# bwohlberg/sporco

Measured on AMD Instinct MI355X. Metric: ConvBPDN ADMM iterations/s, higher is better.
Workload: dtype f32; 1 GPU; admm.cbpdn.ConvBPDN 512x512 greyscale, K=64 8x8 filters, N=32 images per GPU, lambda=0.05, default options (AutoRho, stats every iteration); global_images=32, parallelism=image-shard x1

## Files before the change

sporco_amd/csrc/api_admm_run.inc:

```
    bool admm_run_supported(const sporco_amd_admm_params &p) const {
        return !cplx && std::is_same<T, float>::value && rows_ok && mr_ok(p) && (fused || fused_slabs) && !fused_mc &&
               !tail_mode && !(p.flags & (F_XRRS | F_GRADREG | F_KEEP_X | F_FEVAL_Y)) &&
               (!(p.flags & F_JOINT) || joint_rows_ok(p)) && p.lmbda >= 0.0 && p.rho > 0.0 &&
               !std::getenv("SPORCO_AMD_HOST_LOOP");
    }

    bool persist_ok(const sporco_amd_admm_params &p, const sporco_amd_admm_ctrl &c, bool vf,
                    bool has_reduce) const {
        const bool off = sw.persist >= 0 ? sw.persist != 1 : !hint_one_launch;
        return !off && vf && !has_reduce && fused && !fused_slabs && Ks == K && run_always_emit &&
               admm_persist_supported<T>(H, W, K) && !wl1.ptr && c.max_iter >= 3 &&
               !(p.flags & (F_NOBNDRY | F_AMS | F_JOINT)) && admm_persist_resident<T>(H, W, K, CN);
    }
    PersistIterArgs<T> persist_iter_args(const sporco_amd_admm_params &p, const T *vin, T *vout,
                                         double *prow, double *pcol) {
        PersistIterArgs<T> a;
        cx<T> *Xf = cv(SPORCO_AMD_VAR_XF);
        a.fwd.y = a.fwd.u = nullptr;
        a.fwd.v = vin;
        a.fwd.flags = p.flags;
        a.fwd.C = C;
        a.fwd.N = N;
        a.fwd.dH = p.dH;
        a.fwd.dW = p.dW;
// ... 14 lines not shown
        a.cols.twB = twB;
        a.cols.rho = (T)p.rho;
        a.cols.H = H;
        a.cols.W = W;
        a.cols.CN = CN;
        a.cols.K = K;
        a.cols.partials = pcol;
        a.cols.Ks = Ks;
        a.post.twA = twRows;
        a.post.t_next = Xf;
        a.post.t = Xf;
        a.post.twW = planW.tw<T>();
        a.post.y = a.post.u = nullptr;
        a.post.y_out = a.post.u_out = nullptr;
        a.post.v_in = vin;
        a.post.v_out = vout;
        a.post.x = nullptr;
        a.post.scale = T(1.0 / ((double)H * (double)W));
        a.post.rlx = (T)p.rlx;
        a.post.thr = T(0);
        a.post.u_scale = T(1);
        a.post.flags = p.flags;
        a.post.H = H;
        a.post.W = W;
        a.post.C = C;
        a.post.N = N;
        a.post.K = K;
        a.post.dH = p.dH;
        a.post.dW = p.dW;
        a.post.P = P;
        a.post.Ks = Ks;
        a.post.partials = prow;
        return a;
    }
    int run_persist(const sporco_amd_admm_params &p, int index0, int max_iter, T *v_prev, T *v_other,
                    bool want_sums) {
        const int grid = admm_persist_grid<T>(H, W, K, CN);
        const int64_t nrow = (int64_t)H * ceil_div(P, 128), ncol = (int64_t)Wf * CN;
        if (!pst_part_rows) {
            SA_HIP(hipMalloc((void **)&pst_part_rows, sizeof(double) * 8 * nrow));
            SA_HIP(hipMalloc((void **)&pst_part_f, sizeof(double) * 2 * ncol));
            SA_HIP(hipMalloc((void **)&pst_bar, sizeof(unsigned) * kPersistBarWords));
        }
        if (pst_grid < grid) {
            if (pst_blk) {
                sync();
                SA_HIP(hipFree(pst_blk));
                SA_HIP(hipFree(pst_ctl));
            }
            SA_HIP(hipMalloc(&pst_blk, sizeof(PersistIterArgs<T>) * 2 * grid));
            SA_HIP(hipMalloc((void **)&pst_ctl, sizeof(AdmmCtl) * grid));
            pst_grid = grid;
        }
        AdmmPersistArgs<T> a;
        const int p0 = index0 & 1;
        a.iter[p0] = persist_iter_args(p, v_prev, v_other, part_rows, part_f);
        a.iter[p0 ^ 1] = persist_iter_args(p, v_other, v_prev, pst_part_rows, pst_part_f);
        a.blk = static_cast<PersistIterArgs<T> *>(pst_blk);
        a.ctl_blk = pst_ctl;
        a.ctl = ctl_dev;
        a.rec = reinterpret_cast<AdmmRecord *>(rec_ring) + index0;
        a.index0 = index0;
        a.max_iter = max_iter - index0;
        a.bar = pst_bar;
        a.n_row_tiles = (int)nrow;
        a.n_col_tiles = (int)ncol;
        a.want_dfid = (p.flags & F_OBJ) ? 1 : 0;
        a.want_sums = want_sums ? 1 : 0;
        a.dfid_scale = 1.0 / ((double)H * W);
        SA_HIP(hipMemsetAsync(pst_bar, 0, sizeof(unsigned) * kPersistBarWords, st));
        {
            ProfScope ps(prof, PS_PERSIST);
            launch_admm_persist<T>(st, a, grid);
        }
        unsigned bar[16];
        SA_HIP(hipMemcpyAsync(bar, pst_bar, sizeof(bar), hipMemcpyDeviceToHost, st));
        sync();
        if (bar[2]) throw Error(SPORCO_AMD_EHIP, "one-launch solve: a grid barrier did not complete");
        xf_tiled = true;
        ++pst_runs;
        return (int)bar[3];
    }

    int64_t enqueue_iter_ctl(const sporco_amd_admm_params &p, const T *vin = nullptr,
                             T *vout = nullptr) {
        T *Y = vin ? nullptr : static_cast<T *>(vars[SPORCO_AMD_VAR_Y]);
        T *U = vin ? nullptr : static_cast<T *>(vars[SPORCO_AMD_VAR_U]);
        cx<T> *Xf = cv(SPORCO_AMD_VAR_XF);
        {
            RowsFwdArgs<T> ra;
            ra.y = Y;
            ra.u = U;
            ra.v = vin;
            ra.flags = p.flags;
            ra.C = C;
            ra.N = N;
            if (vin) {
                ra.wl1 = wl1;
                ra.dH = p.dH;
                ra.dW = p.dW;
                ra.ams_bits = ams_bits_of(p);
                ra.ams_k = Ku - 1;
            }
            ra.s2 = T(1);
            ra.t = Xf;
            ra.Ks = Ks;
            ra.twA = twRows;
            ra.H = H;
            ra.W = W;
            ra.CN = CN;
            ra.K = K;
            ra.P = P;
            ra.ctl = ctl_dev;
            ProfScope ps(prof, vin ? PS_ROWS_FWD_V : PS_ROWS_FWD);
            launch_rows_fwd<T>(st, ra);
        }
        {
            FusedColsArgs<T> fa;
            fa.t = Xf;
            fa.dft = dft;
            fa.sft = sft;
            fa.gramt = gramt;
            fa.twA = twA;
            fa.twB = twB;
            fa.rho = (T)p.rho;
            fa.H = H;
            fa.W = W;
            fa.CN = CN;
            fa.K = K;
            fa.partials = part_f;
            fa.Ks = Ks;
            fa.ctl = ctl_dev;
            if (cols_striped() && !fused_slabs) {
                fa.out_even = cols_out[0];
                fa.out_odd = cols_out[1];
            }
            ProfScope ps(prof, PS_FUSED_COLS);
            if (fused_slabs) {
                FusedSlabArgs<T> sa;
                sa.c = fa;
                sa.qpart = qpart;
                part_f_rows = (int)run_slab_cols(sa);
            } else {
                part_f_rows = (int)launch_fused_cols<T>(st, fa);
            }
            xf_tiled = true;
        }
        RowsPostArgs<T> pa;
        pa.twA = twRows;
        pa.t_next = nullptr;
        pa.t = Xf;
        if (cols_striped() && !fused_slabs) {
            pa.t = cols_out[0];
            pa.t_odd = cols_out[1];
        }
        pa.twW = planW.tw<T>();
        pa.y = Y;
        pa.u = U;
        pa.y_out = y_alt;
        pa.u_out = u_alt;
        pa.v_in = vin;
        pa.v_out = vout;
        pa.x = nullptr;
        pa.scale = T(1.0 / ((double)H * (double)W));
        pa.rlx = (T)p.rlx;
        pa.thr = T(0);
        pa.u_scale = T(1);
        pa.flags = p.flags;
        pa.H = H;
        pa.W = W;
        pa.C = C;
        pa.N = N;
        pa.K = K;
        pa.dH = p.dH;
        pa.dW = p.dW;
        pa.P = P;
        pa.wl1 = wl1;
        pa.Ks = Ks;
        pa.ams_bits = ams_bits_of(p);
        pa.ams_k = Ku - 1;
        pa.partials = part_rows;
        pa.ctl = ctl_dev;
        int64_t nt = 0;
        if (!run_always_emit) {
            ProfScope ps(prof, vin ? PS_ROWS_INV_POST_V : PS_ROWS_INV_POST);
            nt = launch_rows_inv_post<T>(st, pa);
        }
        pa.t_next = Xf;
        {
            ProfScope ps(prof, vin ? PS_ROWS_INV_POST_V_EMIT : PS_ROWS_INV_POST_EMIT);
            nt = launch_rows_inv_post<T>(st, pa);
        }
        if (!vout) {
            std::swap(vars[SPORCO_AMD_VAR_Y], reinterpret_cast<void *&>(y_alt));
            std::swap(vars[SPORCO_AMD_VAR_U], reinterpret_cast<void *&>(u_alt));
        }
        return nt;
    }

    int admm_run(const sporco_amd_admm_params &p, const sporco_amd_admm_ctrl &c,
                 sporco_amd_admm_record *records, double *rho_out, double *u_scale_out,
                 sporco_amd_reduce_fn reduce, void *user) override {
        require_ready();
        if (!admm_run_supported(p)) return -1;
        if (gv_live) ensure_yu();
        SA_REQUIRE(c.max_iter >= 0, "max_iter must not be negative");
        if (c.max_iter == 0) {
            *rho_out = p.rho;
            *u_scale_out = p.u_scale;
            return 0;
        }
        if (!y_alt) alloc_alt_pair();
        const bool nn = p.flags & F_NONNEG, jn = p.flags & F_JOINT;
        if (v_live && (!vform_ok(p) || !vform_same_opts(p))) ensure_yu();
        const bool vf = vform_ok(p) && (v_live || c.max_iter >= 4 || hint_vform);
        if (!vf) ensure_yu();
        const bool v_at_entry = v_live;
        T *const v_entry = v_cur;
        const T v_entry_thr = v_thr, v_entry_thr21 = v_thr21;
        if (!ctl_dev) SA_HIP(hipMalloc((void **)&ctl_dev, sizeof(AdmmCtl)));
        if (rec_cap < c.max_iter) {
            if (rec_ring) SA_HIP(hipHostFree(rec_ring));
            rec_cap = std::max(c.max_iter, 256);
            SA_HIP(hipHostMalloc((void **)&rec_ring, sizeof(AdmmRecord) * rec_cap, 0));
        }
        std::memset((void *)rec_ring, 0, sizeof(AdmmRecord) * c.max_iter);
        double *out_dev = out_dev_default;
        const bool want_sums = p.flags & (F_RESID | F_OBJ);
        AdmmCtlInit in;
        in.rho = p.rho;
        in.u_scale = p.u_scale;
        in.lmbda = p.lmbda;
        in.abstol = c.abs_tol;
        in.reltol = c.rel_tol;
        in.sqrt_nc = c.sqrt_nc;
        in.sqrt_nx = c.sqrt_nx;
        in.tau = c.rho_tau;
        in.mu = c.rho_mu;
        in.xi = c.rho_xi;
        in.mu21 = p.mu;
        in.k = c.k0;
        in.stable_run = stable_run;
        in.emitted = t_ready ? 1 : 0;
        in.is_f32 = 1;
        in.autorho = c.auto_rho;
        in.period = c.period > 0 ? c.period : 1;
        in.autoscaling = c.auto_scaling;
        in.stdres = c.std_residuals;
        in.need_resid = c.need_residuals;
        in.thr_prev = v_at_entry ? (float)v_entry_thr : 0.f;
        in.thr21_prev = v_at_entry ? (float)v_entry_thr21 : 0.f;
        in.no_speculation = sw.no_speculation ? 1 : 0;
        run_always_emit = !in.no_speculation && E <= ((int64_t)1 << 22);
        if (run_always_emit) in.no_speculation = 2;
        launch_admm_ctl_init(st, ctl_dev, in);
        SA_HIP(hipMemsetAsync(out_dev, 0, sizeof(double) * kOutSlots, st));
        const int ahead = c.lookahead > 0 ? c.lookahead : 3;
        int enq = 0, done = 0, stop_at = -1;
        int lag = std::getenv("SPORCO_AMD_RUN_LAG") ? std::atoi(std::getenv("SPORCO_AMD_RUN_LAG")) : 0;
        auto poll = [&](int upto, bool block) {
            while (done < upto && stop_at < 0) {
                if (rec_ring[done].seq != done + 1) {
                    if (!block) return;
                    if (hipStreamQuery(st) == hipSuccess && rec_ring[done].seq != done + 1)
                        throw Error(SPORCO_AMD_EHIP, "device-driven solve: record not written");
                    continue;
                }
                if (rec_ring[done].stop) stop_at = done;
                ++done;
            }
        };
        T *vb_in = v_at_entry ? v_entry : nullptr;
        T *const vb_first = vf ? (vb_in == y_alt ? u_alt : y_alt) : nullptr;
        auto enqueue_one = [&]() {
            T *vb_out = vf ? (vb_in == y_alt ? u_alt : y_alt) : nullptr;
            const int64_t nt = enqueue_iter_ctl(p, vb_in, vb_out);
            vb_in = vb_out;
            if (want_sums) {
                const int slots[7] = {SPORCO_AMD_OUT_R2, SPORCO_AMD_OUT_S2, SPORCO_AMD_OUT_AX2,
                                      SPORCO_AMD_OUT_Y2, SPORCO_AMD_OUT_U2, SPORCO_AMD_OUT_L1,
                                      SPORCO_AMD_OUT_L21};
                const double scales[7] = {1, 1, 1, 1, 1, 1, 1};
                const int fslots[2] = {SPORCO_AMD_OUT_DFID, SPORCO_AMD_OUT_RGR};
                const double fscales[2] = {1.0 / ((double)H * W), 1.0 / ((double)H * W)};
                const bool dfid = p.flags & F_OBJ;
                {
                    ProfScope ps(prof, PS_FINALIZE);
                    launch_finalize2(st, part_rows, (int)nt, 8, (p.flags & F_JOINT) ? 7 : 6, slots,
                                     scales, part_f, part_f_rows,
                                     1, dfid ? 1 : 0, fslots, fscales, out_dev);
                }
                if (reduce) reduce(user, out_dev);
                else if (comm_user) comm_reduce_sums(comm_user, out_dev, st);
            }
            launch_admm_ctl_update(st, ctl_dev, out_dev, rec_ring + enq, enq, true);
            ++enq;
        };
        const bool shard = reduce != nullptr || comm_user != nullptr;
        const int wlag = shard ? 0 : lag;
        if (persist_ok(p, c, vf, shard)) {
            enqueue_one();
            T *v0 = vb_in, *v1 = (v0 == y_alt) ? u_alt : y_alt;
            enq += run_persist(p, 1, c.max_iter, v0, v1, want_sums);
            if (c.need_residuals) poll(enq, false);
        }
        for (; enq < c.max_iter && stop_at < 0 && !persist_ok(p, c, vf, shard);) {
            enqueue_one();
            if (c.need_residuals) {
                poll(enq - lag, false);
                if (stop_at < 0 && enq - wlag - done > ahead) poll(enq - wlag - ahead, true);
            }
        }
        if (shard && want_sums && c.need_residuals) {
            if (stop_at < 0) poll(enq, true);
            if (stop_at >= 0)
                while (enq < c.max_iter && enq < stop_at + 1 + ahead) enqueue_one();
        }
        sync();
        poll(enq, false);
        const int n = stop_at >= 0 ? stop_at + 1 : enq;
        if (!vf && ((enq - n) & 1)) {
            std::swap(vars[SPORCO_AMD_VAR_Y], reinterpret_cast<void *&>(y_alt));
            std::swap(vars[SPORCO_AMD_VAR_U], reinterpret_cast<void *&>(u_alt));
        }
        if (vf) {
            T *other_first = vb_first == y_alt ? u_alt : y_alt;
            v_cur = ((n - 1) & 1) ? other_first : vb_first;
            v_thr = (T)(p.lmbda / rec_ring[n - 1].rho);
            v_thr21 = (T)(p.mu / rec_ring[n - 1].rho);
            if (n >= 2) {
                v_prev_kind = 2;
                v_prev_thr = (T)(p.lmbda / rec_ring[n - 2].rho);
                v_prev_thr21 = (T)(p.mu / rec_ring[n - 2].rho);
            } else if (v_at_entry) {
                v_prev_kind = 2;
                v_prev_thr = v_entry_thr;
                v_prev_thr21 = v_entry_thr21;
            } else {
                v_prev_kind = 1;
            }
            v_nonneg = nn;
            v_joint = jn;
            v_opts = p.flags & (F_NOBNDRY | F_AMS);
            v_dH = p.dH;
            v_dW = p.dW;
            v_live = true;
        }
        vp_pending = false;
        AdmmCtl fin;
        SA_HIP(hipMemcpy(&fin, ctl_dev, sizeof(AdmmCtl), hipMemcpyDeviceToHost));
        for (int i = 0; i < n; ++i) {
            const AdmmRecord &r = rec_ring[i];
            sporco_amd_admm_record &o = records[i];
            for (int j = 0; j < kOutSlots; ++j) o.sums[j] = r.sums[j];
            o.r = r.r;
            o.s = r.s;
            o.epri = r.epri;
            o.edua = r.edua;
            o.rho = r.rho;
            o.u_scale = r.u_scale;
            o.seconds = (double)r.ticks * 1e-8;
            o.k = r.k;
            o.stop = r.stop;
        }
        *rho_out = fin.rho;
        *u_scale_out = fin.u_scale;
        stable_run = fin.stable_run > 0 ? fin.stable_run - 1 : 0;
        if (fin.u_scale != 1.0) stable_run = 0;
        t_ready = fin.emitted != 0;
        last_p = p;
        last_p.rho = rec_ring[n - 1].rho;
        last_p.u_scale = rec_ring[n - 1].u_scale;
        x_stale = true;
        x_invalid = p.flags & F_NO_X;
        prev_in_alt = !vf;
        return n;
    }

    void rows_inverse_to(T *Xout, const cx<T> *t_in = nullptr) {
        RowsProxArgs<T> ra;
        ra.t_in = t_in ? t_in : cv(SPORCO_AMD_VAR_XF);
// ... 54 lines not shown
```

sporco_amd/csrc/csc_api.hip:

```cpp
#include "csc_impl.h"

#include <chrono>
#include <string>

namespace sporco_amd {

thread_local std::string g_last_error;
std::atomic<int64_t> g_xfer[4];
const char *kProfNames[PS_COUNT] = {"fft_r2c_rows",     "fft_c2c_cols_fwd", "sm_solve",
                                           "fft_c2c_cols_inv", "fft_c2r_rows",     "admm_post",
                                           "fused_cols_sm",    "rows_fwd",         "rows_inv_post",
                                           "rows_inv_post_emit",
                                           "rows_fwd_v",       "rows_inv_post_v",  "rows_inv_post_v_emit",
                                           "pgm_grad_ifft",    "pgm_rows_prox",    "pgm_fft_momentum",
                                           "finalize",         "pgm_elementwise",  "other",
                                           "admm_persist_run",
                                    "setcoef_rows",     "setcoef_cols",     "ccmod_grad_tiled",
                                    "fft_c2r_vpost",    "fft_c2r_vpost_emit",
                                    "inhib_update"};

struct Switches {
    bool unfused, old_rows, no_pad, no_vform, no_speculation, no_cols_sm, md_generic, cns_generic, cg_host,
        placement_off, placement_force;
    int persist;
    int cols_sm_force_slab;
    static bool set(const char *name) { return std::getenv(name) != nullptr; }
    static Switches read() {
        Switches s;
        s.unfused = set("SPORCO_AMD_UNFUSED");
        s.old_rows = set("SPORCO_AMD_OLD_ROWS");
        s.no_pad = set("SPORCO_AMD_NO_PAD");
        s.no_vform = set("SPORCO_AMD_NO_VFORM");
        s.no_speculation = set("SPORCO_AMD_NO_SPECULATION");
        s.no_cols_sm = set("SPORCO_AMD_NO_COLS_SM");
        s.md_generic = set("SPORCO_AMD_MD_GENERIC");
        s.cns_generic = set("SPORCO_AMD_CNS_GENERIC");
        s.cg_host = set("SPORCO_AMD_CG_HOST");
        const char *e = std::getenv("SPORCO_AMD_PLACEMENT");
        s.placement_off = e && e[0] == '0';
        s.placement_force = e && e[0] == 'f';
        e = std::getenv("SPORCO_AMD_PERSIST");
        s.persist = e ? (e[0] == '1' ? 1 : 0) : -1;
        e = std::getenv("SPORCO_AMD_COLS_SM_FORCE_SLAB");
        s.cols_sm_force_slab = e ? std::atoi(e) : 0;
        return s;
    }
};

template <typename T> struct Csc : CscBase {
    const Switches sw = Switches::read();
    sporco_amd_dims dm;
    int device;
    hipStream_t st = nullptr;
    bool own_stream = false;
    int H, W, Wf, C, N, K, CN;
    int Ku;
    int Cd = 1, Cs, CNs;
    cx<T> *ism_gam = nullptr, *ism_del = nullptr, *ism_mm = nullptr;
    bool fused_mc = false;
    cx<T> *dft_mc = nullptr, *sft_mc = nullptr;
    T *bt_mc = nullptr;
    bool binv_valid = false;
    double binv_rho = 0.0;
    cx<T> *cns_f = nullptr;
    static constexpr int kTailMax = 8;
    int Ks = 0;
    int64_t EFt = 0;
    bool tail_mode = false;
    cx<T> *sft_eff = nullptr, *coef_t = nullptr;
    uint32_t *ams_bits = nullptr;
    bool ams_bits_valid = false;
    T *cns_m = nullptr, *cns_yold = nullptr;
    bool cns_active = false;
    T *md_s = nullptr;
    bool eq_active = false;
    bool zsf_valid = false, dism_valid = false;
    double dism_rho = 0.0;
    cx<T> *dism_gam = nullptr, *dism_del = nullptr, *dism_mm = nullptr;
    T *gramz_t = nullptr;
    bool gramz_valid = false;
    bool cns_fused() const {
        return rows_ok && fused && cols256 && !mr && !sw.cns_generic;
    }
    bool ism_valid = false;
    double ism_rho = 0.0, ism_mu = -1.0;
    int64_t P, E, npix, EF;
    FftPlan planW, planH;
    int depth = 1, Hs = 0;
    FftPlan planD;
    void *vars[SPORCO_AMD_VAR_COUNT] = {nullptr};
    cx<T> *work = nullptr;
    cx<T> *dwork = nullptr;
    T *pcn_stats = nullptr;
    cx<T> *innerb = nullptr;
    T *gram = nullptr;
    T *dpad = nullptr;
    T *sreal = nullptr;
    T *wl1_buf = nullptr, *wl21_buf = nullptr, *wams_buf = nullptr, *wdat_buf = nullptr;
    Weight<T> wl1, wl21, wams;
    Weight<T> wdat;
    bool have_wdat = false;
    double *part_a = nullptr, *part_b = nullptr;
    bool cplx = false;
    cx<T> *df_im = nullptr;
    double *out_dev_own = nullptr;
    double *out_pinned = nullptr;
    bool have_dict = false, have_signal = false;
    int dH_ = 0, dW_ = 0;
    bool fused = false, xf_tiled = false;
    bool cols256 = false;
    bool fused_slabs = false;
    cx<T> *qpart = nullptr;
    unsigned *coop_flags = nullptr;
    unsigned coop_seq = 0;
    int *coop_err = nullptr;
    cx<T> *dft = nullptr, *sft = nullptr, *twA = nullptr, *twB = nullptr;
    T *gramt = nullptr;
    double *part_f = nullptr;
    int part_f_rows = 0;
    bool rows_ok = false;
    bool mr = false;
    bool mr_ok(const sporco_amd_admm_params &p) const {
        return !mr || (Cd == 1 && !wl21.ptr && !(p.flags & F_XRRS));
    }
    cx<T> *twRows = nullptr;
    double *part_rows = nullptr;
    double *pst_part_rows = nullptr, *pst_part_f = nullptr;
    void *pst_blk = nullptr;
    AdmmCtl *pst_ctl = nullptr;
    unsigned *pst_bar = nullptr;
    int pst_grid = 0, pst_runs = 0;
    T *y_alt = nullptr, *u_alt = nullptr;
    bool x_stale = false, x_invalid = false;
    bool md_x_pending = false;
    bool prev_in_alt = false;
    bool v_live = false;
    T *v_cur = nullptr;
    T v_thr = T(0), v_prev_thr = T(0);
    T v_thr21 = T(0), v_prev_thr21 = T(0), vp_thr21 = T(0);
    bool v_nonneg = false, v_joint = false;
    uint32_t v_opts = 0;
    int v_dH = 1, v_dW = 1;
    int v_prev_kind = 0;
    bool vp_pending = false;
    T *vp_buf = nullptr, *vp_free = nullptr;
    T vp_thr = T(0);
    bool vp_nonneg = false;
    uint64_t touch_epoch = 0, fused_epoch = ~(uint64_t)0;
    bool gv_live = false, gv_nonneg = false;
    T gv_thr = T(0);
    uint64_t gen_epoch = ~(uint64_t)0;
    bool t_ready = false;
    int stable_run = 0;
    AdmmCtl *ctl_dev = nullptr;
    AdmmRecord *rec_ring = nullptr;
    int rec_cap = 0;
    CgCtl *cg_dev = nullptr;
    CgPinned *cg_pin = nullptr;
    sporco_amd_admm_params last_p;
    bool zf_tiled = false;
    cx<T> *gpart = nullptr;
    int ccmod_groups = 1;
    bool pgm_tiled = false, pgm_x_stale = false;
    sporco_amd_pgm_params last_pgm;
    double *part_pgm = nullptr, *part_pgm2 = nullptr;
    cx<T> *ccmod_r = nullptr;
    cx<T> *pgm_ey = nullptr;
    bool pgm_held = false;
    bool run_always_emit = false;
    T *ghh = nullptr, *ghw = nullptr, *wg = nullptr;
    bool have_wg = false;
    T *g1t = nullptr;
    bool g1_valid = false;
    double g1_rho = 0.0, g1_mu = 0.0;

    int padded_filters(int H_, int W_, int K_) const {
        if (K_ % 2 == 0 || sw.unfused || sw.no_pad)
            return K_;
        const bool cols = fused_cols_supported<T>(H_, K_ + 1) || fused_slabs_supported<T>(H_, K_ + 1);
        return (cols && rows_supported<T>(W_, K_ + 1)) ? K_ + 1 : K_;
    }

    Csc(const sporco_amd_dims &d, int dev, void *stream, int cd, int depth_ = 1) : dm(d), device(dev) {
        SA_REQUIRE(d.H >= 1 && d.W >= 1 && d.C >= 1 && d.N >= 1 && d.K >= 1,
                   "all dimensions must be >= 1");
        SA_REQUIRE(cd == 1 || cd == d.C,
                   "a multi-channel dictionary needs as many channels as the signal");
        SA_HIP(hipSetDevice(device));
        H = d.H;
        W = d.W;
        Cd = cd;
        Cs = d.C;
        C = cd > 1 ? 1 : d.C;
        N = d.N;
        Ku = d.K;
        K = cd > 1 ? d.K : padded_filters(d.H, d.W, d.K);
        Wf = W / 2 + 1;
        CN = C * N;
        CNs = Cs * N;
        P = (int64_t)C * N * K;
        E = (int64_t)H * W * P;
        npix = (int64_t)H * Wf;
        EF = npix * P;
        if (stream) {
            st = (hipStream_t)stream;
        } else {
            SA_HIP(hipStreamCreate(&st));
            own_stream = true;
        }
        prof.st = st;
        depth = depth_;
        SA_REQUIRE(depth >= 1 && H % depth == 0 && (depth == 1 || cd == 1),
                   "volume handle: depth divides H, single-channel dictionary");
        Hs = H / depth;
        const bool generic_only = sw.unfused || depth > 1;
        planW.init(W);
        planH.init(Hs);
        if (depth > 1) planD.init(depth);
        SA_HIP(hipMalloc((void **)&part_a, sizeof(double) * kMaxPartialBlocks * 8));
        SA_HIP(hipMalloc((void **)&part_b, sizeof(double) * kMaxPartialBlocks * 8));
        SA_HIP(hipMalloc((void **)&out_dev_own, sizeof(double) * kOutSlots));
        SA_HIP(hipMemset(out_dev_own, 0, sizeof(double) * kOutSlots));
        SA_HIP(hipHostMalloc((void **)&out_pinned, sizeof(double) * kOutSlots, 0));
        out_dev_default = out_dev_own;
        SA_HIP(hipMalloc((void **)&gram, sizeof(T) * npix));
        SA_HIP(hipMalloc((void **)&innerb, sizeof(cx<T>) * npix * CNs));
        SA_HIP(hipMalloc((void **)&sreal, sizeof(T) * (int64_t)H * W * CNs));
        fused = Cd == 1 && fused_cols_supported<T>(H, K) && K % 2 == 0 &&
                !generic_only;
        cols256 = H == 128 || H == 256 || H == 512;
        fused_slabs = Cd == 1 && fused_slabs_supported<T>(H, K) && !generic_only;
        fused_mc = Cd > 1 && fused_mc_supported<T>(H, K, Cd) && K % 2 == 0 &&
                   !generic_only;
        if (fused_mc) {
            SA_HIP(hipMalloc((void **)&dft_mc, sizeof(cx<T>) * npix * Cd * K));
            SA_HIP(hipMalloc((void **)&sft_mc, sizeof(cx<T>) * npix * CNs));
            SA_HIP(hipMalloc((void **)&bt_mc, sizeof(T) * npix * 2 * Cd * Cd));
// ... 39 lines not shown
            SA_HIP(hipMalloc((void **)&dft, sizeof(cx<T>) * npix * Ks));
        }
        if (rows_ok) {
            SA_HIP(hipMalloc((void **)&twRows, sizeof(cx<T>) * W));
            std::vector<cx<T>> ta(W);
            rows_twiddles<T>(W, ta.data());
            SA_HIP(hipMemcpy(twRows, ta.data(), sizeof(cx<T>) * W, hipMemcpyHostToDevice));
            SA_HIP(hipMalloc((void **)&part_rows,
                             sizeof(double) * 8 * (int64_t)H *
                                 std::max<int64_t>(ceil_div(P, 128), (int64_t)N * ceil_div(K, 32))));
        }
        for (int v : {SPORCO_AMD_VAR_Y, SPORCO_AMD_VAR_U, SPORCO_AMD_VAR_X}) (void)var_ptr(v);
    }

    std::vector<std::pair<void *, void *>> skew_reg;
    void big_alloc(void **p, size_t bytes) {
        for (size_t i = 0; i < spare_big.size(); ++i)
            if (spare_big[i].second >= bytes && spare_big[i].second <= bytes + bytes / 8) {
                *p = spare_big[i].first;
                spare_big.erase(spare_big.begin() + i);
                spare_vs.erase(spare_vs.begin() + i);
                return;
            }
        big_alloc_fresh(p, bytes);
    }
    void big_alloc_fresh(void **p, size_t bytes) {
        if (bytes >= ((size_t)64 << 20)) {
            const size_t al = (size_t)kAllocAlignMb << 20;
            void *base = nullptr;
            SA_HIP(hipMalloc(&base, bytes + al));
            const uintptr_t b = reinterpret_cast<uintptr_t>(base);
            *p = reinterpret_cast<void *>((b + al - 1) / al * al);
            skew_reg.emplace_back(*p, base);
            return;
        }
        SA_HIP(hipMalloc(p, bytes));
    }
    void big_free(void *p) {
        if (!p) return;
        for (auto &e : skew_reg)
            if (e.first == p) {
                (void)hipFree(e.second);
                e.first = nullptr;
                return;
            }
        (void)hipFree(p);
    }

    ~Csc() override {
        (void)hipSetDevice(device);
        (void)hipStreamSynchronize(st);
        place_release_spares();
        inhib_release();
        big_free(gemit);
        if (part_vpost) (void)hipFree(part_vpost);
        big_free(cols_out[0]);
        big_free(cols_out[1]);
        for (hipEvent_t e : place_ev)
            if (e) (void)hipEventDestroy(e);
        for (auto &v : vars) big_free(v);
        big_free(y_alt);
        big_free(u_alt);
        big_free(work);
        y_alt = u_alt = nullptr;
        work = nullptr;
        for (void *p : {(void *)pst_part_rows, (void *)pst_part_f, pst_blk, (void *)pst_ctl, (void *)pst_bar,
                        (void *)cns_w, (void *)cns_sft, (void *)flt_h, (void *)flt_w,
                        (void *)zf_ch, (void *)zfv_buf, (void *)md_sft, (void *)md_coef, (void *)pgm_rx[0], (void *)pgm_rx[1]})
            if (p) (void)hipFree(p);
        for (void *p : {(void *)dft, (void *)sft, (void *)gramt, (void *)part_f, (void *)twA, (void *)twB,
                        (void *)twRows, (void *)part_rows, (void *)y_alt, (void *)u_alt, (void *)part_pgm, (void *)part_pgm2, (void *)ccmod_r, (void *)pgm_ey, (void *)gpart,
                        (void *)qpart, (void *)coop_flags, (void *)ghh, (void *)ghw, (void *)wg, (void *)g1t, (void *)ism_gam, (void *)ism_del, (void *)ism_mm, (void *)dft_mc, (void *)sft_mc, (void *)bt_mc, (void *)cns_f, (void *)cns_m, (void *)sft_eff, (void *)coef_t, (void *)ams_bits, (void *)gramz_t,
                        (void *)cns_yold, (void *)md_s, (void *)dism_gam, (void *)dism_del, (void *)dism_mm,
                        (void *)dwork, (void *)pcn_stats, (void *)work, (void *)innerb, (void *)gram, (void *)dpad, (void *)sreal,
                        (void *)wl1_buf, (void *)wl21_buf, (void *)wams_buf, (void *)wdat_buf, (void *)part_a, (void *)part_b, (void *)part_cs, (void *)df_im, (void *)pgm_es[0], (void *)pgm_es[1], (void *)pgm_es[2], (void *)pgm_es[3],
                        (void *)out_dev_own})
            if (p) (void)hipFree(p);
        if (out_pinned) (void)hipHostFree(out_pinned);
        if (coop_err) (void)hipHostFree(coop_err);
        if (rec_ring) (void)hipHostFree(rec_ring);
        if (cg_pin) (void)hipHostFree((void *)cg_pin);
        if (cg_dev) (void)hipFree(cg_dev);
        if (ctl_dev) (void)hipFree(ctl_dev);
        planW.destroy();
        planH.destroy();
        if (depth > 1) planD.destroy();
        if (own_stream) (void)hipStreamDestroy(st);
    }

    int64_t KD() const { return (int64_t)Cd * K; }
    static bool var_is_signal_real(int var) {
        return var >= SPORCO_AMD_VAR_MY0 && var <= SPORCO_AMD_VAR_DMU0;
    }
    size_t var_bytes(int var) const {
        if (var == SPORCO_AMD_VAR_SF) return sizeof(cx<T>) * npix * CNs;
        if (var_is_signal_real(var)) return sizeof(T) * (int64_t)H * W * CNs;
        if (var_is_dict_sized(var))
            return var_is_complex(var) ? sizeof(cx<T>) * npix * KD()
                                       : sizeof(T) * (int64_t)H * W * KD();
        if (var == SPORCO_AMD_VAR_CX || var == SPORCO_AMD_VAR_CU) return sizeof(T) * E * Cd;
        return var_is_complex(var) ? sizeof(cx<T>) * EF : sizeof(T) * E;
    }

    size_t var_alloc_bytes(int var) const {
        return var == SPORCO_AMD_VAR_XF ? sizeof(cx<T>) * (size_t)std::max(EF, EFt) : var_bytes(var);
    }
    void *var_ptr(int var) {
        SA_REQUIRE(var_is_valid(var), "unknown state variable id");
        if (var == SPORCO_AMD_VAR_Y || var == SPORCO_AMD_VAR_U) {
            ++touch_epoch;
            if (v_live || gv_live) ensure_yu();
        }
        if (!vars[var]) {
            const size_t nb = var_alloc_bytes(var);
            big_alloc(&vars[var], nb);
            SA_HIP(hipMemsetAsync(vars[var], 0, nb, st));
        }
        return vars[var];
    }
    T *rv(int var) { return static_cast<T *>(var_ptr(var)); }
    cx<T> *cv(int var) { return static_cast<cx<T> *>(var_ptr(var)); }
    cx<T> *work_buf() {
        if (!work) big_alloc((void **)&work, sizeof(cx<T>) * std::max(EF, EFt));
        return work;
    }
    cx<T> *dwork_buf() {
        if (!dwork) SA_HIP(hipMalloc((void **)&dwork, sizeof(cx<T>) * npix * KD()));
        return dwork;
    }
    T *pcn_stats_buf() {
        if (!pcn_stats) SA_HIP(hipMalloc((void **)&pcn_stats, sizeof(T) * 2 * KD()));
        return pcn_stats;
    }
    Dims5 d5() const { return Dims5{H, W, C, N, K}; }

    void *stream_handle() override { return (void *)st; }
    void sync() override {
        SA_HIP(hipStreamSynchronize(st));
        if (coop_err && *coop_err) {
            *coop_err = 0;
            throw Error(SPORCO_AMD_EHIP, "cooperating slab workgroups: a partner's partial sums never "
                                         "arrived; the iterates of this handle are invalid");
        }
    }
    bool pgm_fused_ok() const {
        return rows_ok && (cols256 || mr) && (fused || (fused_slabs && !tail_mode && !mr));
    }
    bool hint_vform = false, hint_one_launch = false;
    bool cplx_pair = false;
    void set_hint(int what, int value) override {
        if (what == SPORCO_AMD_HINT_KEEP_VFORM) hint_vform = value != 0;
        else if (what == SPORCO_AMD_HINT_ONE_LAUNCH) hint_one_launch = value != 0;
        else if (what == SPORCO_AMD_MODE_COMPLEX_PAIR) {
            SA_REQUIRE(Cd == 2 && Cs == 2, "complex pair mode: a handle with two channels (real, imaginary)");
            SA_REQUIRE(!have_signal && !zf_ch, "complex pair mode is set before the signal and the coefficient maps");
            cplx_pair = value != 0;
        } else if (what == SPORCO_AMD_VOLUME_FILTER_DEPTH) {
            SA_REQUIRE(depth > 1 && value >= 1 && value <= depth, "filter depth: a volume handle, 1 <= value <= depth");
            SA_REQUIRE(!flt_h, "volume handle: one filter support (no multi-scale dictionary)");
            vol_dD = value;
        } else throw Error(SPORCO_AMD_EINVAL, "unknown hint");
    }
    void pm_pair(const cx<T> *src, cx<T> *dst, int mid, int inner, int mode) {
        ProfScope ps(prof, PS_OTHER);
        launch_pm_butterfly<T>(st, src, dst, npix, mid, inner, W, mode);
    }
// ... 59 lines not shown
```

sporco_amd/csrc/csc_rows.h:

```cpp
#pragma once

#include "common.h"
#include "csc_fused.h"
#include "csc_kernels.h"

namespace sporco_amd {

template <typename T> struct RowsFwdArgs {
    const T *y, *u;
    T s2;
    cx<T> *t;
    const cx<T> *twA;
    int H, W, CN, K;
    int64_t P;
    const T *v = nullptr;
    T thr_prev = T(0);
    uint32_t flags = 0;
    T thr21_prev = T(0);
    int C = 1, N = 0;
    Weight<T> wl1;
    int dH = 1, dW = 1;
    const uint32_t *ams_bits = nullptr;
    int ams_k = -1;
    int y_bcast = 0;
    int Ks = 0;
    const AdmmCtl *ctl = nullptr;
    int persist = 0;
    int stagger_groups = 1, stagger_sleeps = 0;
};

template <typename T> struct RowsPostArgs {
    const cx<T> *t;
    const cx<T> *t_odd = nullptr;
    const cx<T> *twW;
    const cx<T> *twA;
    cx<T> *t_next;
    int emit_u = 0;
    const T *y, *u;
    T *y_out, *u_out;
    T *x;
    const T *v_in = nullptr;
    T *v_out = nullptr;
    T thr_prev = T(0);
    T thr21_prev = T(0);
    T scale;
    T rlx, thr, u_scale;
    T thr21 = T(0);
    uint32_t flags;
    int H, W, C, N, K, dH, dW;
    int64_t P;
    Weight<T> wl1;
    int Ks = 0;
    const uint32_t *ams_bits = nullptr;
    int ams_k = -1;
    double *partials;
    const AdmmCtl *ctl = nullptr;
    int persist = 0;
    int stagger_groups = 1, stagger_sleeps = 0;
};

template <typename T>
void launch_ams_pack(hipStream_t st, const Weight<T> &mask, uint32_t *bits, int H, int W, int C,
                     int N);

template <typename T> struct RowsProxArgs {
    const cx<T> *t_in;
    cx<T> *t_out;
    T *x;
    const cx<T> *twA, *twW;
    T scale, thr;
    uint32_t flags;
    int H, W, C, N, K, dH, dW;
    int64_t P;
    int Ks = 0;
    Weight<T> wl1;
    double *partials;
    int persist = 0;
    int stagger_groups = 1, stagger_sleeps = 0;
};
template <typename T> int64_t launch_rows_inv_prox_fwd(hipStream_t st, const RowsProxArgs<T> &a);

template <typename T> bool rows_joint_supported(int W, int C, int K);
template <typename T> bool rows_supported(int W, int K);
bool rows_mr_width(int W);
template <typename T> void rows_twiddles(int W, cx<T> *twA);
template <typename T> void launch_rows_fwd(hipStream_t st, const RowsFwdArgs<T> &a);
template <typename T> int64_t launch_rows_inv_post(hipStream_t st, const RowsPostArgs<T> &a);

template <typename T> struct PersistIterArgs {
    RowsFwdArgs<T> fwd;
    FusedColsArgs<T> cols;
    RowsPostArgs<T> post;
};
template <typename T> struct AdmmPersistArgs {
    PersistIterArgs<T> iter[2];
    PersistIterArgs<T> *blk;
    AdmmCtl *ctl_blk;
    AdmmCtl *ctl;
    AdmmRecord *rec;
    int index0, max_iter;
    unsigned *bar;
    int n_row_tiles, n_col_tiles;
    int want_dfid, want_sums;
    double dfid_scale;
};
constexpr int kPersistBarWords = 160;
template <typename T> bool admm_persist_supported(int H, int W, int K);
template <typename T> int admm_persist_grid(int H, int W, int K, int CN);
template <typename T> bool admm_persist_resident(int H, int W, int K, int CN);
template <typename T> void launch_admm_persist(hipStream_t st, const AdmmPersistArgs<T> &a, int grid);

}
```

sporco_amd/csrc/csc_rows_body.inc:

```
#include "csc_rows.h"

#include <cmath>
#include <cstdlib>

#include "csc_ctl_dev.h"
#include "csc_fused_body.h"
#include "regfft.h"

namespace sporco_amd {

namespace {

using namespace regfft;

struct alignas(16) cf2 {
    cf a, b;
};

constexpr int kN1 = 32;
constexpr size_t rows_lds_bytes(int NW) {
    return sizeof(f2) * 16 * NW * 64 + sizeof(double) * 8 * 16;
}

template <int N1, int NW> constexpr int spectral_waves() { return regfft::mr_length(N1) ? (N1 + 1) / 2 : NW; }
// ... 625 lines not shown
                    un[e] = u1;
                    const float dr = xs[e] - y1, ds = y1 - yo[e];
                    s_r2 = sa_fma(dr, dr, s_r2);
                    s_s2 = sa_fma(ds, ds, s_s2);
                    s_x2 = sa_fma(xs[e], xs[e], s_x2);
                    s_y2 = sa_fma(y1, y1, s_y2);
                    s_u2 = sa_fma(u1, u1, s_u2);
                }
                if constexpr (EMIT_T) {
                    SA_VGPR_FENCE3(s_r2, s_s2, s_x2);
                    SA_VGPR_FENCE3(s_y2, s_u2, s_l1);
                }
                const float gv0 = gy ? yn[0] : xs[0], gv1 = gy ? yn[1] : xs[1];
                s_l1 += fabsf(gv0);
                s_l1 += fabsf(gv1);
                float g2[2] = {gv0 * gv0, gv1 * gv1};
                sum_over_rows2(g2[0], g2[1]);
                s_l21 = sa_fma(l21w, sa_sqrt(g2[0]), s_l21);
                s_l21 = sa_fma(l21w, sa_sqrt(g2[1]), s_l21);
                if constexpr (EMIT_T) SA_VGPR_FENCE3(s_l21, s_l1, s_r2);
            } else {
#pragma unroll
            for (int e = 0; e < 2; ++e) {
                const float ax = sa_fma(al, xs[e], oma * yo[e]);
                const bool am = GENERAL && am_e[e];
                const float wt = wte[e];
                const float vv = sa_fma(usc, uraw[e], ax);
                float y1 = soft1_m<MODE>(vv, thr * wt);
                y1 = sa_med3(y1, am ? -__builtin_inff() : nn_lo, __builtin_inff());
                if (GENERAL) y1 *= am ? mkeep : keep;
                const float u1 = vv - y1;
                yn[e] = y1;
                un[e] = u1;
                vn[e] = vv;
                const float dr = xs[e] - y1, ds = y1 - yo[e];
                s_r2 = sa_fma(dr, dr, s_r2);
                s_s2 = sa_fma(ds, ds, s_s2);
                s_x2 = sa_fma(xs[e], xs[e], s_x2);
                s_y2 = sa_fma(y1, y1, s_y2);
                s_u2 = sa_fma(u1, u1, s_u2);
                s_l1 += fabsf(wt * (gy ? y1 : xs[e]));
            }
            }
            if constexpr (VOUT) {
                buf_store_cf(Yo, voff, soff, mk<float>(vn[0], vn[1]));
            } else {
                buf_store_cf(Yo, voff, soff, mk<float>(yn[0], yn[1]));
                buf_store_cf(Uo, voff, soff, mk<float>(un[0], un[1]));
            }

            if (WRITE_X) buf_store_cf(Xb, voff, soff, mk<float>(xs[0], xs[1]));
            if constexpr (EMIT_T && SF == 0) {
                v[n1] = mk<float>(emit_y * yn[0] - emit_s * un[0], emit_y * yn[1] - emit_s * un[1]);
            } else if constexpr (PARK && b * B >= NP) {
                f2 t;
                t.x = yn[0] - un[0];
                t.y = yn[1] - un[1];
                L[((n1 - NP) * NW + w) * 64 + lane] = t;
            } else if (EMIT_T) {
                v[n1] = mk<float>(yn[0] - un[0], yn[1] - un[1]);
            }
        }
    });
    if constexpr (PARK) {
#pragma unroll
        for (int i = 0; i < NP; ++i) {
            const f2 t = L[(i * NW + w) * 64 + lane];
            v[NP + i] = mk<float>(t.x, t.y);
        }
    }

    SA_VGPR_FENCE3(s_r2, s_s2, s_x2);
    SA_VGPR_FENCE3(s_y2, s_u2, s_l1);
    if (EMIT_T) {
        reg_fence<N1>(v, 0, token);
        spatial_to_spectral<NW, COH, N1>(v, a->twA, a->t_next, CN, a->H, a->Ks ? a->Ks : a->K, cn, k, h, pv, w, lane,
                                         L, token);
        __syncthreads();
    }

    double acc[8] = {(double)s_r2, (double)s_s2, (double)s_x2,   (double)s_y2,
                     (double)s_u2, (double)s_l1, (double)s_l21, 0.0};
    const int64_t tile = (int64_t)h * tiles_x + bx;
    block_sum_store<8, COH>(acc, scratch, a->partials + tile * 8);
}

template <int NW, bool WRITE_X, int MODE, bool EMIT_T, bool JOINT = false, int SF = 0, int N1 = kN1>
__global__ void __launch_bounds__(NW * 64, (JOINT && EMIT_T && NW == 8) ? 4 : 1)
rows_inv_post_kernel(const RowsPostArgs<float> a_in) {
    if (a_in.ctl && (a_in.ctl->stop | (a_in.ctl->emit != (EMIT_T ? 1 : 0)))) return;
    const int tiles_x = JOINT ? a_in.N * (a_in.K >> 5) : (int)((a_in.P + 127) / 128);
    rows_tile_loop(a_in, tiles_x, a_in.H, [tiles_x](auto a, int bx, int h) {
        rows_inv_post_tile<NW, WRITE_X, MODE, EMIT_T, JOINT, SF, false, N1>(a, bx, h, tiles_x);
    });
}

template <int NW, bool GENERAL, int N1 = kN1, typename AP>
__device__ __forceinline__ void rows_inv_prox_fwd_tile(AP ap, int bx, int h, int tiles_x) {
    constexpr int W = N1 * NW;
    const auto &a = *ap;
    const int tid = threadIdx.x;
    const int lane = tid & 63;
    const int w = sa_readfirstlane(tid >> 6);
    const int64_t p = (int64_t)bx * 128 + 2 * lane;
    const bool pv = p < a.P;
    const int CN = a.C * a.N;
    const int cn = pv ? (int)(p / a.K) : 0, k = pv ? (int)(p % a.K) : 0;
    f2 *L = dyn_lds<f2>();
    double *scratch = reinterpret_cast<double *>(L + 16 * NW * 64);
    int token = 0;

    cf v[N1];
    spectral_to_spatial<NW, false, N1>(v, a.twW, a.t_in, CN, a.H, a.Ks ? a.Ks : a.K, cn, k, h, pv, w, lane, L,
                                       token);

    const int64_t rowoff = (int64_t)h * W * a.P;
    const uint32_t rowbytes = (uint32_t)((int64_t)W * a.P * sizeof(float));
    const BufRsrc Xb = a.x ? make_rsrc(a.x + rowoff, rowbytes) : make_rsrc(a.t_in, 0u);
    const int voff = pv ? (int)(p * (int64_t)sizeof(float)) : (int)0x80000000;
    const int pixbytes = (int)(a.P * (int64_t)sizeof(float));
    const float scale = a.scale;
    const bool nonneg = a.flags & F_NONNEG, nob = a.flags & F_NOBNDRY;
    int wlane = 0;
    const int ws4 = (int)a.wl1.stride[4];
    if (GENERAL) {
        const int c = cn / a.N, n = cn % a.N;
        wlane = (int)(c * a.wl1.stride[2] + n * a.wl1.stride[3] + k * a.wl1.stride[4]);
    }
    const bool hkill = GENERAL && nob && h >= ((a.dH > 1) ? a.H - (a.dH - 1) : 0);
    const int x0kill = (a.dW > 1) ? W - (a.dW - 1) : 0;
    const float nn_lo = nonneg ? 0.f : -__builtin_inff();
    float s_l1 = 0.f;
#pragma unroll
    for (int n1 = 0; n1 < N1; ++n1) {
        const int xw = NW * n1 + w;
        const float keep = (GENERAL && (hkill || (nob && xw >= x0kill))) ? 0.f : 1.f;
        float y[2] = {v[n1].re * scale, v[n1].im * scale};
#pragma unroll
        for (int e = 0; e < 2; ++e) {
            float wt = 1.f;
            if (GENERAL) {
                const float *wrow = a.wl1.ptr + (int64_t)h * a.wl1.stride[0] +
                                    (int64_t)xw * a.wl1.stride[1];
                wt = wrow[wlane + e * ws4];
            }
            float y1 = GENERAL ? soft1(y[e], a.thr * wt) : soft1_pos(y[e], a.thr);
            y1 = sa_med3(y1, nn_lo, __builtin_inff());
            if (GENERAL) y1 *= keep;
            s_l1 += fabsf(wt * y1);
            y[e] = y1;
        }
        v[n1] = mk<float>(y[0], y[1]);
        buf_store_cf(Xb, voff, xw * pixbytes, v[n1]);
    }
    double acc[1] = {(double)s_l1};
    const int64_t tile = (int64_t)h * tiles_x + bx;
    block_sum_store<1>(acc, scratch, a.partials + tile);
    if (!a.t_out) return;
    reg_fence<N1>(v, 0, token);

    spatial_to_spectral<NW, false, N1>(v, a.twA, a.t_out, CN, a.H, a.Ks ? a.Ks : a.K, cn, k, h, pv, w, lane, L,
                                       token);
}

template <int NW, bool GENERAL, int N1 = kN1>
__global__ void __launch_bounds__(NW * 64) rows_inv_prox_fwd_kernel(const RowsProxArgs<float> a_in) {
    const int tiles_x = (int)((a_in.P + 127) / 128);
    rows_tile_loop(a_in, tiles_x, a_in.H, [tiles_x](auto a, int bx, int h) {
        rows_inv_prox_fwd_tile<NW, GENERAL, N1>(a, bx, h, tiles_x);
    });
}


constexpr int kBarGroup0 = 16, kBarStride = 16;
__device__ __forceinline__ void grid_barrier(unsigned *bar, unsigned nblk) {
    sa_wait_stores();
    __syncthreads();
// ... 250 lines not shown
```

Before: 387.0 iterations/s (512x512, K=64, N=32 per GPU; summed over GPUs).

## Fuse reduction finalize and ADMM control update into rows-inverse-post kernel tail

Adds a last-block-arrives tail to the rows_inv_post kernel. The last block to finish sums the per-tile partials, writes the residual and objective outputs, and runs the ADMM control update on the device. The emit and non-emit variants are merged into one launch that picks the path at run time from ctl->emit. Together these remove the separate reduce/finalize and control-update launches plus the duplicate kernel launch on each iteration. The cost is an atomic arrival counter, a serial reduction done by one block, partial stores made coherent across the grid, and larger kernel code from instantiating both tile paths.

```diff
diff --git a/sporco_amd/csrc/api_admm_run.inc b/sporco_amd/csrc/api_admm_run.inc
--- a/sporco_amd/csrc/api_admm_run.inc
+++ b/sporco_amd/csrc/api_admm_run.inc
@@ -120,8 +120,14 @@
         return (int)bar[3];
     }
 
+    struct TailReq {
+        double *out;
+        AdmmRecord *rec;
+        int index, k;
+        bool want_sums;
+    };
     int64_t enqueue_iter_ctl(const sporco_amd_admm_params &p, const T *vin = nullptr,
-                             T *vout = nullptr) {
+                             T *vout = nullptr, const TailReq *tail = nullptr) {
         T *Y = vin ? nullptr : static_cast<T *>(vars[SPORCO_AMD_VAR_Y]);
         T *U = vin ? nullptr : static_cast<T *>(vars[SPORCO_AMD_VAR_U]);
         cx<T> *Xf = cv(SPORCO_AMD_VAR_XF);
@@ -219,12 +225,28 @@
         pa.ams_k = Ku - 1;
         pa.partials = part_rows;
         pa.ctl = ctl_dev;
+        if (tail) {
+            const bool dfid = p.flags & F_OBJ;
+            pa.tail.arrive = tail_arrive;
+            pa.tail.ctl = ctl_dev;
+            pa.tail.part_f = part_f;
+            pa.tail.part_f_rows = part_f_rows;
+            pa.tail.row_vals = tail->want_sums ? ((p.flags & F_JOINT) ? 7 : 6) : 0;
+            pa.tail.dfid = (tail->want_sums && dfid) ? 1 : 0;
+            pa.tail.dfid_scale = 1.0 / ((double)H * W);
+            pa.tail.out = tail->out;
+            pa.tail.rec = tail->rec;
+            pa.tail.index = tail->index;
+            pa.ctl_k = tail->k;
+        }
+        const bool one_launch = tail && sw.ctl_tail != 2;
         int64_t nt = 0;
-        if (!run_always_emit) {
+        if (!run_always_emit && !one_launch) {
             ProfScope ps(prof, vin ? PS_ROWS_INV_POST_V : PS_ROWS_INV_POST);
             nt = launch_rows_inv_post<T>(st, pa);
         }
         pa.t_next = Xf;
+        pa.emit_rt = (one_launch && !run_always_emit) ? 1 : 0;
         {
             ProfScope ps(prof, vin ? PS_ROWS_INV_POST_V_EMIT : PS_ROWS_INV_POST_EMIT);
             nt = launch_rows_inv_post<T>(st, pa);
@@ -257,6 +279,10 @@
         T *const v_entry = v_cur;
         const T v_entry_thr = v_thr, v_entry_thr21 = v_thr21;
         if (!ctl_dev) SA_HIP(hipMalloc((void **)&ctl_dev, sizeof(AdmmCtl)));
+        if (!tail_arrive) {
+            SA_HIP(hipMalloc((void **)&tail_arrive, sizeof(unsigned) * 2));
+            SA_HIP(hipMemset(tail_arrive, 0, sizeof(unsigned) * 2));
+        }
         if (rec_cap < c.max_iter) {
             if (rec_ring) SA_HIP(hipHostFree(rec_ring));
             rec_cap = std::max(c.max_iter, 256);
@@ -310,10 +336,17 @@
         };
         T *vb_in = v_at_entry ? v_entry : nullptr;
         T *const vb_first = vf ? (vb_in == y_alt ? u_alt : y_alt) : nullptr;
+        const bool shard = reduce != nullptr || comm_user != nullptr;
+        const bool tail_on = !shard && sw.ctl_tail != 0;
         auto enqueue_one = [&]() {
             T *vb_out = vf ? (vb_in == y_alt ? u_alt : y_alt) : nullptr;
-            const int64_t nt = enqueue_iter_ctl(p, vb_in, vb_out);
+            const TailReq tr = {out_dev, rec_ring + enq, enq, c.k0 + enq, want_sums};
+            const int64_t nt = enqueue_iter_ctl(p, vb_in, vb_out, tail_on ? &tr : nullptr);
             vb_in = vb_out;
+            if (tail_on) {
+                ++enq;
+                return;
+            }
             if (want_sums) {
                 const int slots[7] = {SPORCO_AMD_OUT_R2, SPORCO_AMD_OUT_S2, SPORCO_AMD_OUT_AX2,
                                       SPORCO_AMD_OUT_Y2, SPORCO_AMD_OUT_U2, SPORCO_AMD_OUT_L1,
@@ -334,7 +367,6 @@
             launch_admm_ctl_update(st, ctl_dev, out_dev, rec_ring + enq, enq, true);
             ++enq;
         };
-        const bool shard = reduce != nullptr || comm_user != nullptr;
         const int wlag = shard ? 0 : lag;
         if (persist_ok(p, c, vf, shard)) {
             enqueue_one();
diff --git a/sporco_amd/csrc/csc_api.hip b/sporco_amd/csrc/csc_api.hip
--- a/sporco_amd/csrc/csc_api.hip
+++ b/sporco_amd/csrc/csc_api.hip
@@ -24,6 +24,7 @@
         placement_off, placement_force;
     int persist;
     int cols_sm_force_slab;
+    int ctl_tail;
     static bool set(const char *name) { return std::getenv(name) != nullptr; }
     static Switches read() {
         Switches s;
@@ -43,6 +44,8 @@
         s.persist = e ? (e[0] == '1' ? 1 : 0) : -1;
         e = std::getenv("SPORCO_AMD_COLS_SM_FORCE_SLAB");
         s.cols_sm_force_slab = e ? std::atoi(e) : 0;
+        e = std::getenv("SPORCO_AMD_CTL_TAIL");
+        s.ctl_tail = e ? std::atoi(e) : 1;
         return s;
     }
 };
@@ -153,6 +156,7 @@
     bool t_ready = false;
     int stable_run = 0;
     AdmmCtl *ctl_dev = nullptr;
+    unsigned *tail_arrive = nullptr;
     AdmmRecord *rec_ring = nullptr;
     int rec_cap = 0;
     CgCtl *cg_dev = nullptr;
@@ -358,6 +362,7 @@
         if (cg_pin) (void)hipHostFree((void *)cg_pin);
         if (cg_dev) (void)hipFree(cg_dev);
         if (ctl_dev) (void)hipFree(ctl_dev);
+        if (tail_arrive) (void)hipFree(tail_arrive);
         planW.destroy();
         planH.destroy();
         if (depth > 1) planD.destroy();
diff --git a/sporco_amd/csrc/csc_rows.h b/sporco_amd/csrc/csc_rows.h
--- a/sporco_amd/csrc/csc_rows.h
+++ b/sporco_amd/csrc/csc_rows.h
@@ -29,6 +29,19 @@
     int stagger_groups = 1, stagger_sleeps = 0;
 };
 
+struct RowsPostTail {
+    unsigned *arrive = nullptr;
+    AdmmCtl *ctl = nullptr;
+    const double *part_f = nullptr;
+    int part_f_rows = 0;
+    int row_vals = 0;
+    int dfid = 0;
+    double dfid_scale = 0.0;
+    double *out = nullptr;
+    AdmmRecord *rec = nullptr;
+    int index = 0;
+};
+
 template <typename T> struct RowsPostArgs {
     const cx<T> *t;
     const cx<T> *t_odd = nullptr;
@@ -55,6 +68,9 @@
     int ams_k = -1;
     double *partials;
     const AdmmCtl *ctl = nullptr;
+    int emit_rt = 0;
+    int ctl_k = -1;
+    RowsPostTail tail;
     int persist = 0;
     int stagger_groups = 1, stagger_sleeps = 0;
 };
diff --git a/sporco_amd/csrc/csc_rows_body.inc b/sporco_amd/csrc/csc_rows_body.inc
--- a/sporco_amd/csrc/csc_rows_body.inc
+++ b/sporco_amd/csrc/csc_rows_body.inc
@@ -731,17 +731,92 @@
     double acc[8] = {(double)s_r2, (double)s_s2, (double)s_x2,   (double)s_y2,
                      (double)s_u2, (double)s_l1, (double)s_l21, 0.0};
     const int64_t tile = (int64_t)h * tiles_x + bx;
-    block_sum_store<8, COH>(acc, scratch, a->partials + tile * 8);
+    block_sum_store<8, true>(acc, scratch, a->partials + tile * 8);
+}
+
+__device__ __forceinline__ void rows_post_tail(const RowsPostArgs<float> &a_in, int64_t ntiles) {
+    constexpr int FT = kFinalizeThreads;
+    SA_ARGS_PTR_T(RowsPostArgs<float>) a = sa_args_reload(a_in);
+    double *scratch = dyn_lds<double>();
+    double *sums = scratch + 8 * FT;
+    unsigned *flag = reinterpret_cast<unsigned *>(sums + 16);
+    const int tid = threadIdx.x, nth = blockDim.x;
+    unsigned *arrive = a->tail.arrive;
+    if (tid == 0) {
+        const unsigned base = sa_load_agent(arrive + 1);
+        sa_wait_stores();
+        const unsigned n = sa_atomic_inc_agent(arrive) + 1u;
+        flag[0] = (n - base == gridDim.x) ? 1u : 0u;
+        flag[1] = n;
+    }
+    __syncthreads();
+    if (!flag[0]) return;
+    const int nrv = a->tail.row_vals, nv = nrv + (a->tail.dfid ? 1 : 0);
+    const double *prow = a->partials, *pcol = a->tail.part_f;
+    const int ncol = a->tail.part_f_rows;
+    if (tid < 16) sums[tid] = 0.0;
+    for (int idx = tid; idx < nv * FT; idx += nth) {
+        const int v = idx / FT, t = idx % FT;
+        double s = 0.0;
+        if (v < nrv) {
+            int64_t b = t;
+            for (; b + 7 * FT < ntiles; b += 8 * FT) {
+                double q[8];
+#pragma unroll
+                for (int j = 0; j < 8; ++j) q[j] = sa_load_agent(prow + (b + j * FT) * 8 + v);
+#pragma unroll
+                for (int j = 0; j < 8; ++j) s = s + q[j];
+            }
+            for (; b < ntiles; b += FT) s = s + sa_load_agent(prow + b * 8 + v);
+        } else {
+            for (int b = t; b < ncol; b += FT) s = s + pcol[b];
+        }
+        scratch[idx] = s;
+    }
+    __syncthreads();
+    for (int w = FT / 2; w > 0; w >>= 1) {
+        for (int idx = tid; idx < nv * w; idx += nth) {
+            const int v = idx / w, t = idx % w;
+            scratch[v * FT + t] = scratch[v * FT + t] + scratch[v * FT + t + w];
+        }
+        __syncthreads();
+    }
+    if (tid < nv) {
+        const int slots[7] = {SPORCO_AMD_OUT_R2, SPORCO_AMD_OUT_S2, SPORCO_AMD_OUT_AX2, SPORCO_AMD_OUT_Y2,
+                              SPORCO_AMD_OUT_U2, SPORCO_AMD_OUT_L1, SPORCO_AMD_OUT_L21};
+        const int slot = tid < nrv ? slots[tid] : SPORCO_AMD_OUT_DFID;
+        const double r = scratch[tid * FT] * (tid < nrv ? 1.0 : a->tail.dfid_scale);
+        sums[slot] = r;
+        a->tail.out[slot] = r;
+    }
+    __syncthreads();
+    if (tid == 0) {
+        admm_ctl_update_dev<float>(a->tail.ctl, sums, a->tail.rec, a->tail.index);
+        sa_store_agent(arrive + 1, flag[1]);
+    }
 }
 
 template <int NW, bool WRITE_X, int MODE, bool EMIT_T, bool JOINT = false, int SF = 0, int N1 = kN1>
 __global__ void __launch_bounds__(NW * 64, (JOINT && EMIT_T && NW == 8) ? 4 : 1)
 rows_inv_post_kernel(const RowsPostArgs<float> a_in) {
-    if (a_in.ctl && (a_in.ctl->stop | (a_in.ctl->emit != (EMIT_T ? 1 : 0)))) return;
+    if (a_in.ctl) {
+        const AdmmCtl *c = a_in.ctl;
+        if (c->stop | (a_in.ctl_k >= 0 && c->k != a_in.ctl_k)) return;
+        if (!(EMIT_T && a_in.emit_rt) && c->emit != (EMIT_T ? 1 : 0)) return;
+    }
     const int tiles_x = JOINT ? a_in.N * (a_in.K >> 5) : (int)((a_in.P + 127) / 128);
-    rows_tile_loop(a_in, tiles_x, a_in.H, [tiles_x](auto a, int bx, int h) {
-        rows_inv_post_tile<NW, WRITE_X, MODE, EMIT_T, JOINT, SF, false, N1>(a, bx, h, tiles_x);
-    });
+    bool plain = !EMIT_T;
+    if constexpr (EMIT_T) plain = a_in.emit_rt && !a_in.ctl->emit;
+    if (plain) {
+        rows_tile_loop(a_in, tiles_x, a_in.H, [tiles_x](auto a, int bx, int h) {
+            rows_inv_post_tile<NW, WRITE_X, MODE, false, JOINT, SF, false, N1>(a, bx, h, tiles_x);
+        });
+    } else {
+        rows_tile_loop(a_in, tiles_x, a_in.H, [tiles_x](auto a, int bx, int h) {
+            rows_inv_post_tile<NW, WRITE_X, MODE, EMIT_T, JOINT, SF, false, N1>(a, bx, h, tiles_x);
+        });
+    }
+    if (a_in.tail.arrive) rows_post_tail(a_in, (int64_t)tiles_x * a_in.H);
 }
 
 template <int NW, bool GENERAL, int N1 = kN1, typename AP>
```

Result: no change. 386.5 iterations/s (512x512, K=64, N=32 per GPU; summed over GPUs) (-0.1%).
